# HuttleyLab/DiverseSeq

Hardware: AMD Instinct MI355X
Metric: sequences scored/sec (delta-JSD, k=6) (higher is better)
Workload: dtype f64 (results and every set update in f64; reject/accept decisions tiered: f32 and f32-log scores decide rows farther from the threshold than their proven error bands, f64 the rest)

## Files before the change

diverseseq_amd/csrc/api.cpp:

```cpp
#include "dvs_internal.h"

#include <algorithm>
#include <cmath>
#include <cstring>
#include <mutex>

static std::string g_create_err;

int dvs_set_error(dvs_ctx *ctx, int code, const char *fmt, ...) {
    char buf[512];
    va_list ap;
    va_start(ap, fmt);
    vsnprintf(buf, sizeof buf, fmt, ap);
    va_end(ap);
    if (ctx) ctx->err = buf;
    else g_create_err = buf;
    return code;
}

int dvs_hip_fail(dvs_ctx *ctx, hipError_t e, const char *what) {
    (void)hipGetLastError();
    const int code = (e == hipErrorOutOfMemory) ? DVS_ERR_NOMEM : DVS_ERR_RUNTIME;
    return dvs_set_error(ctx, code, "HIP error %d (%s) in %s", int(e), hipGetErrorString(e), what);
}
// ... 45 lines not shown
int dvs_pinned_get(dvs_ctx *ctx, void **ptr) {
    if (!ctx->pinned_pool.empty()) {
        *ptr = ctx->pinned_pool.back();
        ctx->pinned_pool.pop_back();
        if (__builtin_expect(ctx->knobs.test_poison_blocks, 0)) memset(*ptr, 0xFF, 4096);
        return DVS_OK;
    }
    hipError_t e = hipHostMalloc(ptr, 4096, hipHostMallocDefault);
    if (e != hipSuccess) return dvs_hip_fail(ctx, e, "hipHostMalloc");
    if (__builtin_expect(ctx->knobs.test_poison_blocks, 0)) memset(*ptr, 0xFF, 4096);
    return DVS_OK;
}
void dvs_pinned_put(dvs_ctx *ctx, void *ptr) {
    if (!ptr) return;
    if (ctx) ctx->pinned_pool.push_back(ptr);
    else (void)hipHostFree(ptr);
}
hipEvent_t dvs_event_get(dvs_ctx *ctx) {
    if (!ctx->event_pool.empty()) {
        hipEvent_t e = ctx->event_pool.back();
        ctx->event_pool.pop_back();
        return e;
    }
    hipEvent_t e = nullptr;
    (void)hipEventCreate(&e);
    return e;
}
void dvs_event_put(dvs_ctx *ctx, hipEvent_t e) {
    if (!e) return;
    if (ctx) ctx->event_pool.push_back(e);
// ... 150 lines not shown

void dvs_ctx_release(dvs_ctx *ctx) {
    if (!ctx || --ctx->refs > 0) return;
    (void)hipSetDevice(ctx->device);
    dvs_dev_free(ctx, ctx->off_cache.d_off);
    dvs_dev_free(ctx, ctx->off_cache.d_rows);
    dvs_dev_free(ctx, ctx->off_cache.d_tiles);
    if (ctx->off_cache.ev_up) (void)hipEventDestroy(ctx->off_cache.ev_up);
    if (ctx->off_cache.h_off) (void)hipHostFree(ctx->off_cache.h_off);
    if (ctx->pack_ev) (void)hipEventDestroy(ctx->pack_ev);
    if (ctx->h_pack) (void)hipHostFree(ctx->h_pack);
    dvs_dev_free(ctx, ctx->d_clog_tbl);
    for (auto &kv : ctx->canon_reps) dvs_dev_free(ctx, kv.second);
    dvs_dev_trim(ctx);
    for (void *p : ctx->pinned_pool) (void)hipHostFree(p);
    for (hipEvent_t e : ctx->event_pool) (void)hipEventDestroy(e);
    if (ctx->stream2) (void)hipStreamDestroy(ctx->stream2);
    if (ctx->stream_head) (void)hipStreamDestroy(ctx->stream_head);
    if (ctx->stream_rest) (void)hipStreamDestroy(ctx->stream_rest);
    if (ctx->own_stream && ctx->stream) (void)hipStreamDestroy(ctx->stream);
    delete ctx;
}

extern "C" {

const char *dvs_last_error(const dvs_ctx *ctx) { return ctx ? ctx->err.c_str() : g_create_err.c_str(); }

int dvs_ctx_trim(dvs_ctx *ctx) {
    if (!ctx) return DVS_ERR_VALUE;
    dvs_dev_trim(ctx);
// ... 258 lines not shown
```

diverseseq_amd/csrc/dvs_internal.h:

```cpp
#pragma once

#include <hip/hip_runtime.h>

#include <cstdarg>
#include <cstdint>
#include <cstdio>
#include <functional>
#include <map>
#include <string>
#include <vector>

#include "../../include/dvs_hip.h"

#define DVS_EPS 2.220446049250313e-16
#define DVS_HEAD_ROWS 1024u

struct dvs_knobs {
    bool no_uniform_offsets = false;
    bool no_offsets_cache = false;
    bool counts_u32 = false;
    bool build_wait = false;
    bool no_packed_upload = false;
    bool cu_mask_set = false;
    bool no_fast_step = false;
// ... 25 lines not shown
    int device = 0;
    hipStream_t stream = nullptr;
    bool own_stream = false;
    hipStream_t stream2 = nullptr;
    hipStream_t stream_head = nullptr, stream_rest = nullptr;
    int head_cus = 0;
    bool cu_split_tried = false;
    int persist_timeouts = 0;
    int n_cu = 0;
    size_t lds_per_block = 0;
    double *d_clog_tbl = nullptr;
    bool timing = false;
    std::string err;
    std::multimap<size_t, void *> pool;
    std::vector<void *> pinned_pool;
    std::vector<hipEvent_t> event_pool;
    std::map<void *, size_t> live;
    size_t pool_bytes = 0;
    int refs = 1;
    bool owner_gone = false;
    std::map<const void *, size_t> lds_raised;
    std::map<std::pair<const void *, size_t>, bool> persist_fits;
    struct OffsetsCache {
        uint64_t *h_off = nullptr;
        size_t h_cap = 0, n_off = 0;
        hipEvent_t ev_up = nullptr;
        std::vector<uint32_t> h_long_rows;
        std::vector<unsigned char> h_tiles;
        uint64_t nbytes = 0;
        uint32_t k = 0;
// ... 18 lines not shown
struct dvs_matrix;
int dvs_matrix_settle(dvs_ctx *ctx, const dvs_matrix *m);
int dvs_dev_alloc(dvs_ctx *ctx, void **ptr, size_t bytes, const char *what);
void dvs_dev_free(dvs_ctx *ctx, void *ptr);
void dvs_dev_trim(dvs_ctx *ctx);
struct PooledBuf {
    dvs_ctx *ctx;
    void *p = nullptr;
    ~PooledBuf() { dvs_dev_free(ctx, p); }
    template <typename T>
    T *as() { return static_cast<T *>(p); }
};
int dvs_pinned_get(dvs_ctx *ctx, void **ptr);
int dvs_pinned_stage(dvs_ctx *ctx, size_t bytes, const char *what);
void dvs_pinned_put(dvs_ctx *ctx, void *ptr);
hipEvent_t dvs_event_get(dvs_ctx *ctx);
void dvs_event_put(dvs_ctx *ctx, hipEvent_t e);

int dvs_set_error(dvs_ctx *ctx, int code, const char *fmt, ...);
int dvs_hip_fail(dvs_ctx *ctx, hipError_t e, const char *what);

#define DVS_HIP(ctx, call)                                        \
    do {                                                          \
        hipError_t e__ = (call);                                  \
        if (e__ != hipSuccess) return dvs_hip_fail(ctx, e__, #call); \
    } while (0)

struct dvs_matrix {
    int kind = 0;
    uint16_t *d_counts16 = nullptr;
// ... 312 lines not shown
```

diverseseq_amd/csrc/persist.hip:

```cpp
#include "persist_scan.h"
#include "persist_probe.h"

#include <algorithm>
#include <type_traits>
#include <cstddef>
#include <cstdlib>
#include <cstring>

namespace {

template <typename T, bool CACHED, bool MAXM = false, bool SMALL = false>
__global__ __launch_bounds__(P_THREADS, 2) void persist_nmost_kernel(SelDev d, const T *__restrict__ mat,
                                                                    PSync *sync, unsigned long long *part, uint32_t G) {
    static_assert(!SMALL || (CACHED && !MAXM && sizeof(T) == 2), "SMALL: nmost, 16-bit rows, state in the register cache");
    constexpr uint32_t maxn = SMALL ? P_SMALLN : p_maxn(CACHED, MAXM);
    constexpr bool SPEC = CACHED && !MAXM && sizeof(T) <= 4;
    constexpr bool SPEC_BIG = !CACHED && !MAXM && sizeof(T) <= 4;
    constexpr bool OWN = SPEC && !SMALL;
    extern __shared__ __attribute__((aligned(16))) unsigned char smem[];
    const uint64_t B0 = d.B;
    const uint64_t B = B0;
    double *sl = reinterpret_cast<double *>(smem);
    constexpr bool COARSE = CACHED && sizeof(T) <= 4;
    float *slf = reinterpret_cast<float *>(sl + ((B + 1) & ~1ull));
// ... 50 lines not shown
    st.max_size = MAXM ? ctl->max_size : st.n;
    st.stat = ctl->stat;
    st.mean_d = ctl->mean_delta;
    st.std_d = ctl->std_delta;
    st.cov_d = ctl->cov_delta;
    if (lead && tid == 0) ctl->rows_before_launch = ctl->rows_scored;
    if (ctl->status != SEL_RUN || ctl->ev_kind != 0 || st.n > maxn || st.n < 2) {
        if (lead && tid == 0 && ctl->status == SEL_RUN) ctl->why[7]++;
        return;
    }
    if (MAXM && st.n < st.max_size && (ctl->s_is_resum == 0 || st.n + 2 > maxn)) {
        if (lead && tid == 0) ctl->why[6]++;
        return;
    }
    const bool seeded = !MAXM && CACHED && sync->seeded != 0u;
    for (uint32_t r = tid; r < st.n; r += P_THREADS) {
        const uint32_t slot = seeded ? r : d.ord[r];
        const uint64_t mp = seeded ? sync->seed_list[r] : d.mPos[slot];
        const double t = double(d.totals[mp]);
        s_slot[r] = slot;
        s_mH[r] = seeded ? d.rowH[mp] : d.mH[slot];
        s_pos[r] = mp;
        s_tot[r] = t;
        s_rt[r] = 1.0 / t;
    }
    __syncthreads();
    if (!seeded) {
        const double *low = d.M + uint64_t(s_slot[st.li]) * B;
        const double rn0 = 1.0 / double(st.n);
        for (uint64_t i = tid; i < B; i += P_THREADS) {
// ... 257 lines not shown
        for (uint32_t r = 0; r < st.n; r++) {
            const T *mrow = mat + s_pos[r] * B;
            T cv[P_J];
#pragma unroll
            for (int j = 0; j < P_J; j++) cv[j] = mrow[uint64_t(j) * P_THREADS + tid];
            uint4 q;
            q.x = uint32_t(cv[0]) | (uint32_t(cv[1]) << 16);
            q.y = uint32_t(cv[2]) | (uint32_t(cv[3]) << 16);
            q.z = uint32_t(cv[4]) | (uint32_t(cv[5]) << 16);
            q.w = uint32_t(cv[6]) | (uint32_t(cv[7]) << 16);
            *reinterpret_cast<uint4 *>(s_rows + uint64_t(s_slot[r]) * 4096 + uint32_t(tid) * 8) = q;
        }
    }
    if (sync->no_coarse & 2u) st.thr = 1e300;
#ifdef DVS_PERSIST_STAMPS
    unsigned long long *s_dbg = reinterpret_cast<unsigned long long *>(smem + sync->lds_bytes - 128);
    if (tid < 16) s_dbg[tid] = 0ull;
    __syncthreads();
    unsigned long long t_prev = __builtin_amdgcn_s_memrealtime();
#endif
    for (;;) {
        uint64_t B = B0;
        int tid = tid0;
        asm volatile("" : "+s"(B));
        asm volatile("" : "+v"(tid));
        const uint32_t lane = uint32_t(tid) & 63u, wave = uint32_t(tid) >> 6;
        if (epoch >= P_EPOCH_MAX) {
            bail = true;
            break;
        }
        PRel *myrel = &sync->rel[blockIdx.x & 7u];
// ... 1513 lines not shown
    }

#ifdef DVS_PERSIST_STAMPS
#ifdef DVS_PROBE
    if ((blockIdx.x == n_work - 1 || blockIdx.x == 0) && tid == 0)
        for (int k_ = 0; k_ < 16; k_++) (blockIdx.x == 0 ? sync->dbg2 : sync->dbg)[k_] += s_dbg[k_];
#else
    if ((lead || blockIdx.x == 0) && tid == 0)
        for (int k_ = 0; k_ < 16; k_++) (lead ? sync->dbg : sync->dbg2)[k_] += s_dbg[k_];
#endif
#endif
    if (lead && exit_status != SEL_ERROR && !(exit_status == SEL_ARBITER && arb_stage == ARB_FINALIZE)) {
        const double dn_x = double(st.n);
        for (uint64_t i = tid; i < B; i += P_THREADS) d.base[i] = sl[i] / dn_x;
    }
    if (lane == 0 && nread) {
        atomicAdd(&ctl->rows_scored, (unsigned long long)nread);
        if (nprecise) atomicAdd(&ctl->rows_rechecked, (unsigned long long)nprecise);
        if (nmid) atomicAdd(&ctl->rows_coarse_passed, (unsigned long long)nmid);
    }
    if (lead && tid == 0) {
        ctl->cursor = st.cursor;
        ctl->window = st.window < ctl->window_max ? st.window : ctl->window_max;
        ctl->n_windows += st.n_windows;
        ctl->n_events += st.n_events;
        ctl->n_accepts += st.n_accepts;
        ctl->ev_kind = pend_kind;
        if (exit_status == SEL_ARBITER) {
            ctl->arb_stage = arb_stage;
            ctl->arb_pos = arb_pos;
            if (arb_stage == ARB_RESOLVE) ctl->event_pos = arb_pos;
        }
        ctl->status = (bail || (head_phase && exit_status == SEL_DONE)) ? SEL_RUN
                      : (exit_status == SEL_RUN ? SEL_ERROR : exit_status);
// ... 154 lines not shown
}

}

template <typename T>
static const void *persist_fn(const dvs_select *s) {
    const bool cached = s->dev.B <= uint64_t(P_J) * P_THREADS;
    if (s->params.mode == DVS_MODE_MAX) return reinterpret_cast<const void *>(persist_nmost_kernel<T, true, true>);
    if constexpr (std::is_same_v<T, uint16_t>) {
        if (s->persist.small) return reinterpret_cast<const void *>(persist_nmost_kernel<T, true, false, true>);
    }
    return cached ? reinterpret_cast<const void *>(persist_nmost_kernel<T, true>)
                  : reinterpret_cast<const void *>(persist_nmost_kernel<T, false>);
}

static int persist_prepare(dvs_ctx *ctx, dvs_select *s, uint32_t head_stop, hipStream_t on) {
    std::vector<unsigned char> &image = head_stop ? s->persist.h_sync_head : s->persist.h_sync;
    image.assign(sizeof(PSync), 0);
    PSync &init = *reinterpret_cast<PSync *>(image.data());
    init.stop_at = head_stop;
    init.seeded = s->persist.seeded ? 1u : 0u;
    init.seed_list = static_cast<const unsigned long long *>(s->d_seed_list);
    for (int g = 0; g < 8; g++) init.rel[g].hint = ~0ull;
    init.wg_thresh = s->params.window ? 0u : 4u;
    init.wg_scale = 1.5f;
    if (ctx->knobs.persist_wg_rounds >= 0) init.wg_thresh = uint32_t(ctx->knobs.persist_wg_rounds);
    init.no_coarse = (ctx->knobs.persist_no_coarse ? 1u : 0u) | (ctx->knobs.persist_no_events ? 2u : 0u);
    init.small_rows = s->persist.small ? s->persist.small_rows : 0u;
    init.lds_bytes = uint32_t(s->persist.lds);
    init.wmax = uint32_t(std::min<uint64_t>(s->npos, 0xFFFFFFFFull));
    DVS_HIP(ctx, hipMemcpyAsync(head_stop ? s->persist.sync_head : s->persist.sync, &init, sizeof init, hipMemcpyHostToDevice, on));
    DVS_HIP(ctx, hipMemsetAsync(head_stop ? s->persist.part_head : s->persist.part, 0, p_acc_bytes(s->persist.maxn), on));
    return DVS_OK;
}

template <typename T>
static int persist_launch(dvs_ctx *ctx, dvs_select *s, const T *mat, uint32_t grid, uint32_t head_stop,
                          hipStream_t on) {
    const SelDev &d = s->dev;
    if (head_stop ? !s->persist.head_prepared : !s->persist.prepared) {
        int prc = persist_prepare(ctx, s, head_stop, on);
        if (prc) return prc;
    }
    if (head_stop) s->persist.head_prepared = false;
    else s->persist.prepared = false;
    s->persist.seeded = false;
    const hipEvent_t e1 = dvs_scan_timing_start(ctx, s, on);
// ... 44 lines not shown
        return persist_fn<T>(s);
    });
    int rc = dvs_raise_dyn_lds(ctx, fn, lds);
    if (rc) return rc;
    {
        auto key = std::make_pair(fn, lds);
        auto hit = ctx->persist_fits.find(key);
        if (hit == ctx->persist_fits.end()) {
            int per_cu = 0;
            const bool fits = hipOccupancyMaxActiveBlocksPerMultiprocessor(&per_cu, fn, P_THREADS, lds) == hipSuccess && per_cu >= 1;
            if (!fits) (void)hipGetLastError();
            hit = ctx->persist_fits.emplace(key, fits).first;
        }
        if (!hit->second) return DVS_OK;
    }
    rc = dvs_dev_alloc(ctx, &s->persist.sync, sizeof(PSync), "persistent sync block");
    if (!rc) rc = dvs_dev_alloc(ctx, &s->persist.part, p_acc_bytes(s->persist.maxn) + (maxm ? 2 * p_batch_bytes() : 0),
                                "leave-one-out accumulators");
    if (rc) return rc;
    s->persist.on = true;
    return DVS_OK;
}

void dvs_persist_free(dvs_select *s) {
    dvs_dev_free(s->ctx, s->persist.sync);
    dvs_dev_free(s->ctx, s->persist.part);
    dvs_dev_free(s->ctx, s->persist.sync_head);
    dvs_dev_free(s->ctx, s->persist.part_head);
}

int dvs_persist_launch(dvs_ctx *ctx, dvs_select *s) {
    return dvs_mat_dispatch(s->mat, [&](auto *mp) { return persist_launch(ctx, s, mp, s->persist.grid, 0u, ctx->stream); });
}

static int persist_head_blocks(dvs_ctx *ctx, dvs_select *s) {
    if (s->persist.sync_head) return DVS_OK;
    int rc = dvs_dev_alloc(ctx, &s->persist.sync_head, sizeof(PSync), "head phase sync block");
    if (!rc) rc = dvs_dev_alloc(ctx, &s->persist.part_head, p_acc_bytes(s->persist.maxn), "head phase accumulators");
    return rc;
}

int dvs_persist_launch_head(dvs_ctx *ctx, dvs_select *s, uint32_t grid, uint32_t stop_at, hipStream_t on) {
    int rc = persist_head_blocks(ctx, s);
    if (rc) return rc;
    return dvs_mat_dispatch(s->mat, [&](auto *mp) { return persist_launch(ctx, s, mp, grid, stop_at, on); });
}

int dvs_persist_prepare_head(dvs_ctx *ctx, dvs_select *s, uint32_t stop_at, hipStream_t on) {
    int rc = persist_head_blocks(ctx, s);
    if (!rc) rc = persist_prepare(ctx, s, stop_at, on);
    if (!rc) s->persist.head_prepared = true;
    return rc;
}
// ... 43 lines not shown
```

diverseseq_amd/csrc/persist_dev.h:

```cpp
#pragma once

#include "select_dev.h"

namespace {

constexpr int P_THREADS = 512;
constexpr int P_J = 8;
constexpr int P_CH = 16;
constexpr uint32_t P_MAXN = 512;
constexpr uint32_t P_MAXN_BIG = 256;
constexpr uint32_t P_MAXN_MAX = 896;
constexpr uint32_t p_maxn(bool cached, bool maxm = false) { return cached ? (maxm ? P_MAXN_MAX : P_MAXN) : P_MAXN_BIG; }
constexpr uint32_t P_SMALLN = 16;
constexpr uint32_t P_SMALL_ROWS = 13;
constexpr uint32_t p_maxjobs(bool cached, bool maxm = false) { return p_maxn(cached, maxm) + 1; }
constexpr size_t p_acc_bytes(uint32_t maxn) { return size_t(8) * (maxn + 1) * 2 * sizeof(unsigned long long); }
__device__ __forceinline__ unsigned long long p_acc_word(double v) {
    return ((unsigned long long)__double2ll_rn(v * 0x1p50) << 6) + 1ull;
}
__device__ __forceinline__ double p_acc_value(unsigned long long w) { return double((long long)w >> 6) * 0x1p-50; }
__device__ __forceinline__ void p_acc_add(unsigned long long *dst, double th, double ts) {
    atomicAdd(dst, p_acc_word(th));
    atomicAdd(dst + 1, p_acc_word(ts));
}
// ... 12 lines not shown
        v = __hip_atomic_load(w, __ATOMIC_RELAXED, __HIP_MEMORY_SCOPE_AGENT);
    }
    *prev = v;
    return v - before;
}
constexpr uint32_t P_SPIN_LIMIT = 1u << 22;
constexpr uint32_t P_MAXG = 256;
constexpr uint32_t P_FLAT_GRID = 64;
constexpr uint32_t P_WINWORDS = 64;
constexpr uint32_t P_LIST = 2;
constexpr uint32_t P_BATCH = 32;
constexpr uint32_t P_BATCH_MEMBERS = 256;
constexpr size_t p_batch_bytes() { return size_t(P_BATCH) * (P_BATCH_MEMBERS + 2) * 4 * sizeof(double); }
constexpr size_t p_batch_lds() { return size_t(P_BATCH) * (2 + 12 + 24) * sizeof(double); }

constexpr size_t P_LDS_SLACK = 56;
constexpr size_t P_LDS_SLACK_SMALL = 16;
constexpr size_t p_lds_bytes(uint64_t B, int kind, bool cached, bool maxm, uint32_t small_rows) {
    const bool coarse = cached && kind != 1, own = coarse && !maxm && !small_rows;
    const size_t maxn = small_rows ? P_SMALLN : p_maxn(cached, maxm);
    const size_t sl = ((B + 1) & ~1ull) * sizeof(double);
    const size_t slf = coarse ? ((B + 3) & ~3ull) * sizeof(float) : 0;
    const size_t Sl = maxm ? sl : 0;
    const size_t scratch = 128 * sizeof(double);
    const size_t members = maxn * (5 * sizeof(double) + sizeof(uint64_t) + sizeof(uint32_t));
    const size_t s_win = P_WINWORDS * sizeof(unsigned long long), flags = 16, s_ltab = 128 * sizeof(double2);
    const size_t s_prev = (maxn + 1) * 2 * sizeof(unsigned long long);
    const size_t tail = maxm         ? p_batch_lds()
                        : small_rows ? small_rows * B * sizeof(uint16_t) + P_LDS_SLACK_SMALL
                        : own        ? maxn * sizeof(uint32_t) + size_t(P_J) * P_THREADS * (kind == 2 ? sizeof(uint16_t) : sizeof(uint32_t))
                                     : 0;
    const size_t stamps = 128;
    return sl + slf + Sl + scratch + members + s_win + flags + s_ltab + s_prev + tail + stamps + P_LDS_SLACK;
}
static_assert(p_lds_bytes(4096, 2, true, false, 2) == 70440 && p_lds_bytes(4096, 2, true, false, 13) == 160552, "nmost, 4096 bins, 16-bit, SMALL");
static_assert(p_lds_bytes(4096, 2, true, false, 0) == 98008, "nmost, 4096 bins, 16-bit, OWN");
static_assert(p_lds_bytes(4096, 0, true, false, 0) == 106200 && p_lds_bytes(4096, 1, true, false, 0) == 71384, "nmost, 4096 bins, 32-bit and f64");
static_assert(p_lds_bytes(16384, 2, false, false, 0) == 152280 && p_lds_bytes(16384, 0, false, false, 0) == 152280, "nmost, 16384 bins");
static_assert(p_lds_bytes(4096, 2, true, true, 0) == 156376 && p_lds_bytes(256, 2, true, true, 0) == 79576, "max, 16-bit");
static_assert(p_lds_bytes(125, 0, true, false, 0) == 58568, "nmost, 125 bins, 32-bit");

struct PLine {
    uint32_t v;
    uint32_t pad[63];
};
struct PRel {
    unsigned long long rel;
    unsigned long long hint;
// ... 14 lines not shown
    const unsigned long long *seed_list;
    uint32_t small_rows;
    uint32_t lds_bytes;
    uint32_t wmax;
    uint32_t pad2[53];
    PRel rel[8];
    unsigned long long wrec[2][P_MAXG];
    unsigned long long soft[2][P_MAXG][P_LIST];
#ifdef DVS_PERSIST_STAMPS
    unsigned long long trace[4][8][P_MAXG];
#endif
    unsigned long long dbg2[16];
    unsigned long long dbg[16];
};

struct PState {
    uint64_t cursor, npos;
    uint32_t window, wmin, wmax;
    uint32_t n, li;
    double sumH, total_jsd, thr, band, wscale;
    uint32_t n_windows, n_events, n_accepts;
    uint32_t max_size, stat;
    double mean_d, std_d, cov_d;
};

#define RLX_AGENT __ATOMIC_RELAXED, __HIP_MEMORY_SCOPE_AGENT

constexpr uint32_t P_TAG0 = 0xFFFFFEu;
constexpr uint32_t P_EPOCH_MAX = 0xFFFFF0u;
constexpr unsigned long long P_POS_NONE = (1ull << 37) - 1;
// ... 216 lines not shown
```

diverseseq_amd/csrc/select.h:

```cpp
#pragma once

#include "dvs_internal.h"

#define SEL_NONE 0xFFFFFFFFFFFFFFFFull
#define SEL_SEEDS_AT 512

enum : uint32_t { SEL_RUN = 0, SEL_DONE = 1, SEL_ARBITER = 2, SEL_ERROR = 3,
                  SEL_NEED_SETUP = 4 };
enum : uint32_t { ARB_RESOLVE = 1, ARB_FINALIZE = 2 };
enum : uint32_t { FORCE_NONE = 0, FORCE_ACCEPT = 1, FORCE_REJECT = 2, FORCE_COMMIT = 3, FORCE_ROLLBACK = 4 };

struct SelCtl {
    unsigned long long cursor;
    unsigned long long npos;
    unsigned long long event_pos;
    unsigned long long arb_pos;
    unsigned long long rows_scored, rows_rechecked;
    unsigned long long rows_coarse_passed;
    unsigned long long rows_before_launch;
    uint32_t window, window_min, window_max;
    uint32_t status, arb_stage, forced, forced_lowest;
    uint32_t size, lowest, mode, max_size, stat;
    uint32_t ev_kind;
    uint32_t ev_n;
// ... 32 lines not shown
    double *dtmp = nullptr;
    double *dsum = nullptr;
    uint32_t *mLabel = nullptr;
    unsigned long long *mPos = nullptr;
    uint32_t *ord = nullptr;
    uint8_t *inset = nullptr;
    uint32_t *wg_rows = nullptr;
    unsigned long long *evlog_pos = nullptr;
    uint32_t *evlog_kind = nullptr;
    const double *gather_all = nullptr;
    uint32_t gather_world = 0;
    double *rowlog = nullptr;
    uint32_t rowlog_cap = 0;
};

struct dvs_select {
    dvs_ctx *ctx = nullptr;
    dvs_select_params params{};
    const dvs_matrix *mat = nullptr;
    int mat_kind = 0;
    uint64_t npos = 0;
    uint32_t cap = 0;
    SelDev dev;
    SelCtl *h_ctl = nullptr;
    SelCtl ctl0{};
    std::vector<uint32_t> h_order, h_labels;
    std::vector<uint32_t> h_out_labels;
    std::vector<uint64_t> seed_positions;
    uint32_t scan_grid = 0, loo_grid = 0;
    size_t scan_lds = 0;
    bool base_in_lds = true;
    bool scan_hot = false;
    struct {
        bool on = false;
        uint32_t grid = 0, maxn = 0, maxjobs = 0;
        bool small = false;
        uint32_t small_rows = 0;
        size_t lds = 0;
        void *sync = nullptr;
        std::vector<unsigned char> h_sync;
        std::vector<unsigned char> h_sync_head;
        void *part = nullptr;
        void *sync_head = nullptr, *part_head = nullptr;
        bool seeded = false;
        bool head_prepared = false;
        bool prepared = false;
    } persist;
    struct {
        double *d_res = nullptr;
        uint32_t jw = 0;
        uint32_t launched = 0;
    } mb;
    bool seeded_start = false;
    bool used_side_streams = false;
    hipEvent_t ev_side_done = nullptr;
    void *d_seed_list = nullptr;
    bool seed_list_in_ctl = false;
    bool inset_clean = false;
    hipStream_t setup_side = nullptr;
    bool head_phase = false;
    int batch = 16;
    bool time_scan = false;
    std::vector<hipEvent_t> ev_pool;
    size_t ev_used = 0;
    double scan_ms = 0.0;
    double scan_ms_last = 0.0;
    uint64_t scan_launches = 0;
    uint32_t n_arbitrated = 0;
    double arbiter_ms = 0.0;
// ... 13 lines not shown
        uint64_t rowlog_have = 0;
        uint32_t steps_since_poll = 0;
    } fs;
    void *arbiter = nullptr;
};

int dvs_select_arbitrate(dvs_ctx *ctx, dvs_select *s);
void dvs_select_arbiter_free(dvs_select *s);

int dvs_persist_setup(dvs_ctx *ctx, dvs_select *s);
void dvs_persist_free(dvs_select *s);
int dvs_persist_launch(dvs_ctx *ctx, dvs_select *s);
int dvs_persist_launch_head(dvs_ctx *ctx, dvs_select *s, uint32_t grid, uint32_t stop_at, hipStream_t on);
int dvs_persist_prepare_main(dvs_ctx *ctx, dvs_select *s);
int dvs_persist_prepare_head(dvs_ctx *ctx, dvs_select *s, uint32_t stop_at, hipStream_t on);
void dvs_persist_debug_report(dvs_ctx *ctx, const dvs_select *s);
void dvs_persist_debug_done(const SelCtl &c);

hipEvent_t dvs_scan_timing_start(dvs_ctx *ctx, dvs_select *s, hipStream_t on);
void dvs_select_launch_scan(dvs_ctx *ctx, dvs_select *s, bool hot);
void dvs_select_launch_iteration(dvs_ctx *ctx, dvs_select *s, int stage);
int dvs_select_poll(dvs_ctx *ctx, dvs_select *s);
int dvs_select_arbitrate_resume(dvs_ctx *ctx, dvs_select *s);

int dvs_stepwise_alloc(dvs_ctx *ctx, dvs_select *s, const uint32_t *labels);
void dvs_stepwise_wait(dvs_select *s);
void dvs_stepwise_free(dvs_select *s);
#ifdef DVS_FS_TRACE
void dvs_stepwise_trace_report(const dvs_select *s);
#endif
// ... 4 lines not shown
```

diverseseq_amd/csrc/select.hip:

```cpp
#include "dvs_internal.h"
#include "select.h"
#include "select_dev.h"

#include <algorithm>
#include <chrono>
#include <type_traits>
#include <cmath>
#include <cstring>
#include <cstdlib>
#include <memory>

namespace {

constexpr int SCAN_THREADS = 512;

template <typename T>
__device__ __forceinline__ void scan_rows_hot(SelCtl *ctl, const T *__restrict__ mat,
                                              const uint32_t *__restrict__ totals,
                                              const double *__restrict__ rowH, const double *bvec,
                                              uint64_t B, const ScanState &st, uint64_t first,
                                              uint64_t stride, uint32_t lane, uint32_t &nread,
                                              uint32_t &nprecise) {
    for (uint64_t r = first; r < st.nrows; r += stride) {
        const uint64_t p = st.cursor + r;
// ... 685 lines not shown
        for (uint64_t i = threadIdx.x; i < d.B; i += LOO_THREADS) out[i] = 0.0;
        if (threadIdx.x == 0) meta[2 * r] = meta[2 * r + 1] = 0.0;
        return;
    }
    const uint32_t slot = d.ord[r];
    const double *src = d.M + uint64_t(slot) * d.B;
    for (uint64_t i = threadIdx.x; i < d.B; i += LOO_THREADS) out[i] = src[i];
    if (threadIdx.x == 0) {
        meta[2 * r] = double(d.mPos[slot]);
        meta[2 * r + 1] = 1.0;
    }
}

}

static void sel_free(dvs_select *s) {
    if (!s) return;
#ifdef DVS_FS_TRACE
    dvs_stepwise_trace_report(s);
#endif
    if (s->used_side_streams && s->ctx) {
        if (s->ctx->stream_head) (void)hipStreamSynchronize(s->ctx->stream_head);
        if (s->ctx->stream2) (void)hipStreamSynchronize(s->ctx->stream2);
    }
    void *ptrs[] = {s->dev.ctl, s->dev.S, s->dev.Stmp, s->dev.base, s->dev.cand, s->dev.M,
                    s->dev.mH, s->dev.mDelta, s->dev.dtmp, s->dev.dsum, s->dev.mLabel, s->dev.mPos,
                    s->dev.ord, s->dev.inset, s->dev.wg_rows, s->dev.evlog_pos, s->dev.evlog_kind, s->dev.rowlog,
                    (void *)s->dev.order, (void *)s->dev.labels};
    for (void *p : ptrs)
        dvs_dev_free(s->ctx, p);
    dvs_stepwise_wait(s);
    dvs_pinned_put(s->ctx, s->h_ctl);
    for (hipEvent_t e : s->ev_pool) dvs_event_put(s->ctx, e);
    dvs_max_batch_free(s);
    dvs_stepwise_free(s);
    dvs_persist_free(s);
    if (!s->seed_list_in_ctl) dvs_dev_free(s->ctx, s->d_seed_list);
    if (s->ev_side_done) dvs_event_put(s->ctx, s->ev_side_done);
    dvs_select_arbiter_free(s);
    dvs_ctx_release(s->ctx);
    delete s;
}
// ... 48 lines not shown
    hipLaunchKernelGGL(finalize_kernel, dim3(1), dim3(WIDE_THREADS), 0, stream, d);
}

void dvs_select_launch_scan(dvs_ctx *ctx, dvs_select *s, bool hot) {
    dvs_mat_dispatch(s->mat, [&](auto *mp) { launch_scan(s, mp, hot, s->dev.ctl, s->dev.wg_rows, ctx->stream); return 0; });
}
void dvs_select_launch_iteration(dvs_ctx *ctx, dvs_select *s, int stage) {
    dvs_mat_dispatch(s->mat, [&](auto *mp) { launch_iteration(ctx, s, mp, stage); return 0; });
}

int dvs_select_poll(dvs_ctx *ctx, dvs_select *s) {
    DVS_HIP(ctx, hipMemcpyAsync(s->h_ctl, s->dev.ctl, sizeof(SelCtl), hipMemcpyDeviceToHost,
                                ctx->stream));
    DVS_HIP(ctx, hipStreamSynchronize(ctx->stream));
    const_cast<dvs_matrix *>(s->mat)->in_flight = false;
    return DVS_OK;
}

template <typename T>
static int sel_seed(dvs_ctx *ctx, dvs_select *s, const T *mat, hipStream_t st, bool light = false);

template <typename T>
static int sel_drop_seeded(dvs_ctx *ctx, dvs_select *s, const T *mat, hipStream_t st) {
    s->seeded_start = false;
    s->persist.seeded = false;
    return sel_seed<T>(ctx, s, mat, st);
}

template <typename T>
static int sel_leave_persist(dvs_ctx *ctx, dvs_select *s, const T *mat, bool restart) {
// ... 123 lines not shown
    if (s->mat->head_rows_built && s->params.n_seed <= s->mat->head_rows_built && s->h_order.empty() &&
        !(s->params.flags & DVS_SELECT_STEPWISE)) {
        s->head_phase = s->mat->rest_beside_head && ctx->stream_head && s->persist.on &&
                        s->params.mode == DVS_MODE_NMOST && s->params.window == 0 &&
                        s->cap + 2 <= uint32_t(ctx->head_cus) && s->npos > 4ull * s->mat->head_rows_built &&
                        s->params.n_seed + 64 <= s->mat->head_rows_built && !ctx->knobs.no_head_phase;
        s->setup_side = s->head_phase ? ctx->stream_head : dvs_ctx_stream2(ctx);
    }
}

template <typename T>
static int sel_start(dvs_ctx *ctx, dvs_select *s, const T *mat) {
    hipStream_t side = s->setup_side;
    const bool head_phase = s->head_phase;
    hipStream_t st = side ? side : ctx->stream;
    if (side) s->used_side_streams = true;
    int rc = sel_seed<T>(ctx, s, mat, st, s->seeded_start);
    if (rc) return rc;
    if (head_phase) {
        rc = dvs_persist_launch_head(ctx, s, uint32_t(ctx->head_cus), s->mat->head_rows_built, side);
        if (rc == DVS_ERR_UNSUPPORTED)
            rc = s->seeded_start ? sel_drop_seeded<T>(ctx, s, mat, st) : DVS_OK;
        if (rc) return rc;
        rc = dvs_persist_prepare_main(ctx, s);
        if (rc) return rc;
        const_cast<dvs_matrix *>(s->mat)->rest_beside_head = false;
    }
    if (side) {
        if (!s->ev_side_done) s->ev_side_done = dvs_event_get(ctx);
        DVS_HIP(ctx, hipEventRecord(s->ev_side_done, side));
        DVS_HIP(ctx, hipStreamWaitEvent(ctx->stream, s->ev_side_done, 0));
    }
    if (s->params.flags & DVS_SELECT_STEPWISE) return dvs_select_poll(ctx, s);
    return sel_run_loop<T>(ctx, s, mat);
}

template <typename T>
static int sel_seed(dvs_ctx *ctx, dvs_select *s, const T *mat, hipStream_t st, bool light) {
    const std::vector<uint64_t> &seeds = s->seed_positions;
    SelDev &d = s->dev;
    SelCtl c = s->ctl0;
    const uint32_t wdef = s->params.window ? s->params.window : (s->persist.on ? s->persist.grid * 2u : 4096u);
    c.window_min = wdef;
    c.window_max = std::max<uint32_t>(wdef, s->scan_grid * (SCAN_THREADS / 64) * 8);
    c.window = wdef;
    *s->h_ctl = c;
// ... 127 lines not shown
    const struct { void **ptr; size_t bytes; const char *what; } blocks[] = {
        {(void **)&d.ctl, 4096, "d.ctl"},
        {(void **)&d.S, B * 8, "d.S"},
        {(void **)&d.Stmp, B * 8, "d.Stmp"},
        {(void **)&d.base, B * 8, "d.base"},
        {(void **)&d.cand, B * 8, "d.cand"},
        {(void **)&d.M, size_t(cap) * B * 8, "d.M"},
        {(void **)&d.mH, size_t(cap) * 8, "d.mH"},
        {(void **)&d.mDelta, size_t(cap) * 8, "d.mDelta"},
        {(void **)&d.dtmp, size_t(cap) * 8, "d.dtmp"},
        {(void **)&d.dsum, size_t(cap) * 8, "d.dsum"},
        {(void **)&d.mLabel, size_t(cap) * 4, "d.mLabel"},
        {(void **)&d.mPos, size_t(cap) * 8, "d.mPos"},
        {(void **)&d.ord, size_t(cap) * 4, "d.ord"},
        {(void **)&d.inset, std::max<size_t>(nlabels, 1), "d.inset"},
        {(void **)&d.wg_rows, size_t(s->scan_grid) * 8, "d.wg_rows"},
        {(void **)&d.evlog_pos, nlog * 8, "d.evlog_pos"},
        {(void **)&d.evlog_kind, nlog * 4, "d.evlog_kind"},
    };
    for (const auto &b : blocks)
        if (int rc = dvs_dev_alloc(ctx, b.ptr, b.bytes, b.what)) return rc;
    if (s->params.flags & DVS_SELECT_STEPWISE)
        if (int rc = dvs_stepwise_alloc(ctx, s, labels)) return rc;
    if (order) {
        if (int rc = dvs_dev_alloc(ctx, (void **)&d.order, size_t(npos) * 4, "d.order")) return rc;
        DVS_HIP(ctx, hipMemcpyAsync((void *)d.order, order, size_t(npos) * 4, hipMemcpyHostToDevice, ctx->stream));
    }
    if (labels) {
        if (int rc = dvs_dev_alloc(ctx, (void **)&d.labels, size_t(npos) * 4, "d.labels")) return rc;
        DVS_HIP(ctx, hipMemcpyAsync((void *)d.labels, labels, size_t(npos) * 4, hipMemcpyHostToDevice, ctx->stream));
    }
    static_assert(sizeof(SelCtl) <= 4096, "control block must fit a cached pinned block");
    return dvs_pinned_get(ctx, (void **)&s->h_ctl);
}

static int sel_prepare_engine(dvs_ctx *ctx, dvs_select *s, const uint32_t *order, const uint32_t *labels) {
    SelDev &d = s->dev;
    const dvs_matrix *m = s->mat;
    const uint32_t n_seed = s->params.n_seed, nlabels = d.nlabels;
    int rc = dvs_persist_setup(ctx, s);
    if (rc) return rc;
    sel_plan_setup_stream(ctx, s);
    if (s->setup_side) s->used_side_streams = true;
    DVS_HIP(ctx, hipMemsetAsync(d.inset, 0, std::max<size_t>(nlabels, 1), s->setup_side ? s->setup_side : ctx->stream));
    s->inset_clean = true;
    DVS_HIP(ctx, hipMemsetAsync(d.wg_rows, 0, size_t(s->scan_grid) * 8, s->setup_side ? s->setup_side : ctx->stream));
    s->seeded_start = s->persist.on && s->params.mode == DVS_MODE_NMOST && d.B <= 4096 && !order && !labels &&
                      !(s->params.flags & DVS_SELECT_STEPWISE) && n_seed >= 2 && n_seed <= 32 && !ctx->knobs.persist_no_seeded;
    s->persist.seeded = s->seeded_start;
    if (size_t(n_seed) * sizeof(uint64_t) <= 4096 - SEL_SEEDS_AT) {
        s->d_seed_list = reinterpret_cast<unsigned char *>(d.ctl) + SEL_SEEDS_AT;
        s->seed_list_in_ctl = true;
    } else if (s->seeded_start) {
        if ((rc = dvs_dev_alloc(ctx, &s->d_seed_list, size_t(n_seed) * sizeof(uint64_t), "seed list"))) return rc;
    }
    if (s->persist.on && m->rest_beside_head && ctx->stream_head && m->head_rows_built && s->params.mode == DVS_MODE_NMOST &&
        !order && !labels) {
        s->used_side_streams = true;
        return dvs_persist_prepare_head(ctx, s, m->head_rows_built, ctx->stream_head);
    }
    return DVS_OK;
}

static int sel_read_seeds(dvs_ctx *ctx, dvs_select *s, const uint32_t *order) {
    const dvs_matrix *m = s->mat;
    const uint32_t n_seed = s->params.n_seed;
    std::vector<uint32_t> h_tot(n_seed);
    int rc = dvs_matrix_settle(ctx, m);
    if (rc) return rc;
    hipError_t ce = hipSuccess;
    if (!order && n_seed && n_seed <= m->h_head_totals.size()) {
        std::copy(m->h_head_totals.begin(), m->h_head_totals.begin() + n_seed, h_tot.begin());
    } else if (!order && n_seed) {
// ... 239 lines not shown
```

Before: 69.94 million.

## Merge persistent launch blocks into one pinned upload and aggregate exit counters per workgroup

The sync block, the accumulators and (for the head phase) the wg_rows scratch now sit in one device allocation. Each is initialised by a single async copy from a cached, pre-zeroed pinned host image, replacing a separate memcpy plus memsets. Kernel exit counters are first summed in LDS per workgroup, so only one global atomic per counter is issued per workgroup. Side-stream synchronisation at free is skipped for streams already joined, and the head phase reuses its timing event as the join point. The cost is more state tracking, such as pending-upload flags and side-stream bitmasks, plus a change to the LDS layout.

```diff
diff --git a/diverseseq_amd/csrc/api.cpp b/diverseseq_amd/csrc/api.cpp
--- a/diverseseq_amd/csrc/api.cpp
+++ b/diverseseq_amd/csrc/api.cpp
@@ -83,6 +83,27 @@
 void dvs_pinned_put(dvs_ctx *ctx, void *ptr) {
     if (!ptr) return;
     if (ctx) ctx->pinned_pool.push_back(ptr);
+    else (void)hipHostFree(ptr);
+}
+int dvs_pinned_image_get(dvs_ctx *ctx, size_t bytes, void **ptr) {
+    const size_t sz = ((bytes ? bytes : 1) + 4095) & ~size_t(4095);
+    auto it = ctx->pinned_images.find(sz);
+    if (it != ctx->pinned_images.end()) {
+        *ptr = it->second;
+        ctx->pinned_images.erase(it);
+    } else {
+        const hipError_t e = hipHostMalloc(ptr, sz, hipHostMallocDefault);
+        if (e != hipSuccess) {
+            *ptr = nullptr;
+            return dvs_hip_fail(ctx, e, "pinned image of a launch block");
+        }
+    }
+    if (__builtin_expect(ctx->knobs.test_poison_blocks, 0)) memset(*ptr, 0xFF, sz);
+    return DVS_OK;
+}
+void dvs_pinned_image_put(dvs_ctx *ctx, void *ptr, size_t bytes) {
+    if (!ptr) return;
+    if (ctx) ctx->pinned_images.emplace(((bytes ? bytes : 1) + 4095) & ~size_t(4095), ptr);
     else (void)hipHostFree(ptr);
 }
 hipEvent_t dvs_event_get(dvs_ctx *ctx) {
@@ -263,6 +284,7 @@
     for (auto &kv : ctx->canon_reps) dvs_dev_free(ctx, kv.second);
     dvs_dev_trim(ctx);
     for (void *p : ctx->pinned_pool) (void)hipHostFree(p);
+    for (auto &kv : ctx->pinned_images) (void)hipHostFree(kv.second);
     for (hipEvent_t e : ctx->event_pool) (void)hipEventDestroy(e);
     if (ctx->stream2) (void)hipStreamDestroy(ctx->stream2);
     if (ctx->stream_head) (void)hipStreamDestroy(ctx->stream_head);
diff --git a/diverseseq_amd/csrc/dvs_internal.h b/diverseseq_amd/csrc/dvs_internal.h
--- a/diverseseq_amd/csrc/dvs_internal.h
+++ b/diverseseq_amd/csrc/dvs_internal.h
@@ -63,6 +63,7 @@
     std::string err;
     std::multimap<size_t, void *> pool;
     std::vector<void *> pinned_pool;
+    std::multimap<size_t, void *> pinned_images;
     std::vector<hipEvent_t> event_pool;
     std::map<void *, size_t> live;
     size_t pool_bytes = 0;
@@ -111,6 +112,8 @@
 int dvs_pinned_get(dvs_ctx *ctx, void **ptr);
 int dvs_pinned_stage(dvs_ctx *ctx, size_t bytes, const char *what);
 void dvs_pinned_put(dvs_ctx *ctx, void *ptr);
+int dvs_pinned_image_get(dvs_ctx *ctx, size_t bytes, void **ptr);
+void dvs_pinned_image_put(dvs_ctx *ctx, void *ptr, size_t bytes);
 hipEvent_t dvs_event_get(dvs_ctx *ctx);
 void dvs_event_put(dvs_ctx *ctx, hipEvent_t e);
 
diff --git a/diverseseq_amd/csrc/persist.hip b/diverseseq_amd/csrc/persist.hip
--- a/diverseseq_amd/csrc/persist.hip
+++ b/diverseseq_amd/csrc/persist.hip
@@ -88,6 +88,7 @@
         return;
     }
     const bool seeded = !MAXM && CACHED && sync->seeded != 0u;
+    if (tid < 4) p_exit_words(smem, sync)[tid] = 0ull;
     for (uint32_t r = tid; r < st.n; r += P_THREADS) {
         const uint32_t slot = seeded ? r : d.ord[r];
         const uint64_t mp = seeded ? sync->seed_list[r] : d.mPos[slot];
@@ -375,7 +376,7 @@
     }
     if (sync->no_coarse & 2u) st.thr = 1e300;
 #ifdef DVS_PERSIST_STAMPS
-    unsigned long long *s_dbg = reinterpret_cast<unsigned long long *>(smem + sync->lds_bytes - 128);
+    unsigned long long *s_dbg = reinterpret_cast<unsigned long long *>(smem + sync->lds_bytes - P_LDS_STAMPS);
     if (tid < 16) s_dbg[tid] = 0ull;
     __syncthreads();
     unsigned long long t_prev = __builtin_amdgcn_s_memrealtime();
@@ -1919,10 +1920,20 @@
         const double dn_x = double(st.n);
         for (uint64_t i = tid; i < B; i += P_THREADS) d.base[i] = sl[i] / dn_x;
     }
-    if (lane == 0 && nread) {
-        atomicAdd(&ctl->rows_scored, (unsigned long long)nread);
-        if (nprecise) atomicAdd(&ctl->rows_rechecked, (unsigned long long)nprecise);
-        if (nmid) atomicAdd(&ctl->rows_coarse_passed, (unsigned long long)nmid);
+    if (lane == 0) {
+        unsigned long long *s_exit = p_exit_words(smem, sync);
+        if (nread) atomicAdd(&s_exit[0], (unsigned long long)nread);
+        if (nprecise) atomicAdd(&s_exit[1], (unsigned long long)nprecise);
+        if (nmid) atomicAdd(&s_exit[2], (unsigned long long)nmid);
+        const unsigned long long before = __hip_atomic_fetch_add(&s_exit[3], 1ull, __ATOMIC_ACQ_REL, __HIP_MEMORY_SCOPE_WORKGROUP);
+        if (before == P_THREADS / 64 - 1) {
+            const unsigned long long wg_read = __hip_atomic_load(&s_exit[0], __ATOMIC_RELAXED, __HIP_MEMORY_SCOPE_WORKGROUP);
+            const unsigned long long wg_precise = __hip_atomic_load(&s_exit[1], __ATOMIC_RELAXED, __HIP_MEMORY_SCOPE_WORKGROUP);
+            const unsigned long long wg_mid = __hip_atomic_load(&s_exit[2], __ATOMIC_RELAXED, __HIP_MEMORY_SCOPE_WORKGROUP);
+            if (wg_read) atomicAdd(&ctl->rows_scored, wg_read);
+            if (wg_precise) atomicAdd(&ctl->rows_rechecked, wg_precise);
+            if (wg_mid) atomicAdd(&ctl->rows_coarse_passed, wg_mid);
+        }
     }
     if (lead && tid == 0) {
         ctl->cursor = st.cursor;
@@ -2107,23 +2118,35 @@
                   : reinterpret_cast<const void *>(persist_nmost_kernel<T, false>);
 }
 
+static size_t p_block_acc_at() { return (sizeof(PSync) + 255) & ~size_t(255); }
+static size_t p_block_tail_at(uint32_t maxn) { return p_block_acc_at() + p_acc_bytes(maxn); }
+
 static int persist_prepare(dvs_ctx *ctx, dvs_select *s, uint32_t head_stop, hipStream_t on) {
-    std::vector<unsigned char> &image = head_stop ? s->persist.h_sync_head : s->persist.h_sync;
-    image.assign(sizeof(PSync), 0);
-    PSync &init = *reinterpret_cast<PSync *>(image.data());
+    auto &ps = s->persist;
+    void *&image = head_stop ? ps.h_image_head : ps.h_image;
+    size_t &bytes = head_stop ? ps.image_head_bytes : ps.image_bytes;
+    bool &zeroed = head_stop ? ps.image_head_zeroed : ps.image_zeroed;
+    if (!image) {
+        bytes = p_block_tail_at(ps.maxn) + (head_stop ? ps.head_tail : 0);
+        if (int rc = dvs_pinned_image_get(ctx, bytes, &image)) return rc;
+        zeroed = false;
+    }
+    std::memset(image, 0, zeroed ? sizeof(PSync) : bytes);
+    zeroed = true;
+    PSync &init = *static_cast<PSync *>(image);
     init.stop_at = head_stop;
-    init.seeded = s->persist.seeded ? 1u : 0u;
+    init.seeded = ps.seeded ? 1u : 0u;
     init.seed_list = static_cast<const unsigned long long *>(s->d_seed_list);
     for (int g = 0; g < 8; g++) init.rel[g].hint = ~0ull;
     init.wg_thresh = s->params.window ? 0u : 4u;
     init.wg_scale = 1.5f;
     if (ctx->knobs.persist_wg_rounds >= 0) init.wg_thresh = uint32_t(ctx->knobs.persist_wg_rounds);
     init.no_coarse = (ctx->knobs.persist_no_coarse ? 1u : 0u) | (ctx->knobs.persist_no_events ? 2u : 0u);
-    init.small_rows = s->persist.small ? s->persist.small_rows : 0u;
-    init.lds_bytes = uint32_t(s->persist.lds);
+    init.small_rows = ps.small ? ps.small_rows : 0u;
+    init.lds_bytes = uint32_t(ps.lds);
     init.wmax = uint32_t(std::min<uint64_t>(s->npos, 0xFFFFFFFFull));
-    DVS_HIP(ctx, hipMemcpyAsync(head_stop ? s->persist.sync_head : s->persist.sync, &init, sizeof init, hipMemcpyHostToDevice, on));
-    DVS_HIP(ctx, hipMemsetAsync(head_stop ? s->persist.part_head : s->persist.part, 0, p_acc_bytes(s->persist.maxn), on));
+    if (on == ctx->stream) ps.upload_pending = true;
+    DVS_HIP(ctx, hipMemcpyAsync(head_stop ? ps.sync_head : ps.sync, image, bytes, hipMemcpyHostToDevice, on));
     return DVS_OK;
 }
 
@@ -2198,19 +2221,22 @@
         }
         if (!hit->second) return DVS_OK;
     }
-    rc = dvs_dev_alloc(ctx, &s->persist.sync, sizeof(PSync), "persistent sync block");
-    if (!rc) rc = dvs_dev_alloc(ctx, &s->persist.part, p_acc_bytes(s->persist.maxn) + (maxm ? 2 * p_batch_bytes() : 0),
-                                "leave-one-out accumulators");
+    rc = dvs_dev_alloc(ctx, &s->persist.sync, p_block_tail_at(s->persist.maxn) + (maxm ? 2 * p_batch_bytes() : 0),
+                       "persistent launch block");
     if (rc) return rc;
+    s->persist.part = static_cast<unsigned char *>(s->persist.sync) + p_block_acc_at();
     s->persist.on = true;
     return DVS_OK;
 }
 
 void dvs_persist_free(dvs_select *s) {
+    if (s->persist.upload_pending && s->ctx) (void)hipStreamSynchronize(s->ctx->stream);
+    s->persist.upload_pending = false;
     dvs_dev_free(s->ctx, s->persist.sync);
-    dvs_dev_free(s->ctx, s->persist.part);
     dvs_dev_free(s->ctx, s->persist.sync_head);
-    dvs_dev_free(s->ctx, s->persist.part_head);
+    dvs_pinned_image_put(s->ctx, s->persist.h_image, s->persist.image_bytes);
+    dvs_pinned_image_put(s->ctx, s->persist.h_image_head, s->persist.image_head_bytes);
+    s->persist.h_image = s->persist.h_image_head = nullptr;
 }
 
 int dvs_persist_launch(dvs_ctx *ctx, dvs_select *s) {
@@ -2219,8 +2245,17 @@
 
 static int persist_head_blocks(dvs_ctx *ctx, dvs_select *s) {
     if (s->persist.sync_head) return DVS_OK;
-    int rc = dvs_dev_alloc(ctx, &s->persist.sync_head, sizeof(PSync), "head phase sync block");
-    if (!rc) rc = dvs_dev_alloc(ctx, &s->persist.part_head, p_acc_bytes(s->persist.maxn), "head phase accumulators");
+    const int rc = dvs_dev_alloc(ctx, &s->persist.sync_head, p_block_tail_at(s->persist.maxn) + s->persist.head_tail,
+                                 "head phase launch block");
+    if (!rc) s->persist.part_head = static_cast<unsigned char *>(s->persist.sync_head) + p_block_acc_at();
+    return rc;
+}
+
+int dvs_persist_head_tail(dvs_ctx *ctx, dvs_select *s, size_t bytes, void **tail) {
+    if (s->persist.sync_head) return dvs_set_error(ctx, DVS_ERR_RUNTIME, "the head phase's block exists already");
+    s->persist.head_tail = bytes;
+    const int rc = persist_head_blocks(ctx, s);
+    if (!rc) *tail = static_cast<unsigned char *>(s->persist.sync_head) + p_block_tail_at(s->persist.maxn);
     return rc;
 }
 
diff --git a/diverseseq_amd/csrc/persist_dev.h b/diverseseq_amd/csrc/persist_dev.h
--- a/diverseseq_amd/csrc/persist_dev.h
+++ b/diverseseq_amd/csrc/persist_dev.h
@@ -50,7 +50,9 @@
 constexpr size_t p_batch_bytes() { return size_t(P_BATCH) * (P_BATCH_MEMBERS + 2) * 4 * sizeof(double); }
 constexpr size_t p_batch_lds() { return size_t(P_BATCH) * (2 + 12 + 24) * sizeof(double); }
 
-constexpr size_t P_LDS_SLACK = 56;
+constexpr size_t P_LDS_EXIT = 32;
+constexpr size_t P_LDS_STAMPS = 128;
+constexpr size_t P_LDS_SLACK = 24;
 constexpr size_t P_LDS_SLACK_SMALL = 16;
 constexpr size_t p_lds_bytes(uint64_t B, int kind, bool cached, bool maxm, uint32_t small_rows) {
     const bool coarse = cached && kind != 1, own = coarse && !maxm && !small_rows;
@@ -66,8 +68,7 @@
                         : small_rows ? small_rows * B * sizeof(uint16_t) + P_LDS_SLACK_SMALL
                         : own        ? maxn * sizeof(uint32_t) + size_t(P_J) * P_THREADS * (kind == 2 ? sizeof(uint16_t) : sizeof(uint32_t))
                                      : 0;
-    const size_t stamps = 128;
-    return sl + slf + Sl + scratch + members + s_win + flags + s_ltab + s_prev + tail + stamps + P_LDS_SLACK;
+    return sl + slf + Sl + scratch + members + s_win + flags + s_ltab + s_prev + tail + P_LDS_SLACK + P_LDS_EXIT + P_LDS_STAMPS;
 }
 static_assert(p_lds_bytes(4096, 2, true, false, 2) == 70440 && p_lds_bytes(4096, 2, true, false, 13) == 160552, "nmost, 4096 bins, 16-bit, SMALL");
 static_assert(p_lds_bytes(4096, 2, true, false, 0) == 98008, "nmost, 4096 bins, 16-bit, OWN");
@@ -112,6 +113,10 @@
     unsigned long long dbg[16];
 };
 
+__device__ __forceinline__ unsigned long long *p_exit_words(unsigned char *smem, const PSync *sync) {
+    return reinterpret_cast<unsigned long long *>(smem + sync->lds_bytes - (P_LDS_STAMPS + P_LDS_EXIT));
+}
+
 struct PState {
     uint64_t cursor, npos;
     uint32_t window, wmin, wmax;
diff --git a/diverseseq_amd/csrc/select.h b/diverseseq_amd/csrc/select.h
--- a/diverseseq_amd/csrc/select.h
+++ b/diverseseq_amd/csrc/select.h
@@ -70,6 +70,8 @@
     uint32_t rowlog_cap = 0;
 };
 
+constexpr uint8_t SEL_SIDE_HEAD = 1, SEL_SIDE_2 = 2;
+
 struct dvs_select {
     dvs_ctx *ctx = nullptr;
     dvs_select_params params{};
@@ -94,10 +96,14 @@
         uint32_t small_rows = 0;
         size_t lds = 0;
         void *sync = nullptr;
-        std::vector<unsigned char> h_sync;
-        std::vector<unsigned char> h_sync_head;
         void *part = nullptr;
         void *sync_head = nullptr, *part_head = nullptr;
+        void *h_image = nullptr, *h_image_head = nullptr;
+        size_t image_bytes = 0, image_head_bytes = 0;
+        bool image_zeroed = false, image_head_zeroed = false;
+        bool upload_pending = false;
+        size_t head_tail = 0;
+        bool wg_rows_in_head = false;
         bool seeded = false;
         bool head_prepared = false;
         bool prepared = false;
@@ -109,6 +115,7 @@
     } mb;
     bool seeded_start = false;
     bool used_side_streams = false;
+    uint8_t side_open = 0, side_joined = 0;
     hipEvent_t ev_side_done = nullptr;
     void *d_seed_list = nullptr;
     bool seed_list_in_ctl = false;
@@ -152,6 +159,7 @@
 int dvs_persist_launch_head(dvs_ctx *ctx, dvs_select *s, uint32_t grid, uint32_t stop_at, hipStream_t on);
 int dvs_persist_prepare_main(dvs_ctx *ctx, dvs_select *s);
 int dvs_persist_prepare_head(dvs_ctx *ctx, dvs_select *s, uint32_t stop_at, hipStream_t on);
+int dvs_persist_head_tail(dvs_ctx *ctx, dvs_select *s, size_t bytes, void **tail);
 void dvs_persist_debug_report(dvs_ctx *ctx, const dvs_select *s);
 void dvs_persist_debug_done(const SelCtl &c);
 
diff --git a/diverseseq_amd/csrc/select.hip b/diverseseq_amd/csrc/select.hip
--- a/diverseseq_amd/csrc/select.hip
+++ b/diverseseq_amd/csrc/select.hip
@@ -723,18 +723,25 @@
 
 }
 
+static void sel_side_queued(dvs_ctx *ctx, dvs_select *s, hipStream_t st) {
+    const uint8_t bit = st == ctx->stream_head ? SEL_SIDE_HEAD : SEL_SIDE_2;
+    s->used_side_streams = true;
+    s->side_open |= bit;
+    s->side_joined &= uint8_t(~bit);
+}
+
 static void sel_free(dvs_select *s) {
     if (!s) return;
 #ifdef DVS_FS_TRACE
     dvs_stepwise_trace_report(s);
 #endif
     if (s->used_side_streams && s->ctx) {
-        if (s->ctx->stream_head) (void)hipStreamSynchronize(s->ctx->stream_head);
-        if (s->ctx->stream2) (void)hipStreamSynchronize(s->ctx->stream2);
+        if (s->ctx->stream_head && (s->side_open & SEL_SIDE_HEAD)) (void)hipStreamSynchronize(s->ctx->stream_head);
+        if (s->ctx->stream2 && (s->side_open & SEL_SIDE_2)) (void)hipStreamSynchronize(s->ctx->stream2);
     }
     void *ptrs[] = {s->dev.ctl, s->dev.S, s->dev.Stmp, s->dev.base, s->dev.cand, s->dev.M,
                     s->dev.mH, s->dev.mDelta, s->dev.dtmp, s->dev.dsum, s->dev.mLabel, s->dev.mPos,
-                    s->dev.ord, s->dev.inset, s->dev.wg_rows, s->dev.evlog_pos, s->dev.evlog_kind, s->dev.rowlog,
+                    s->dev.ord, s->dev.inset, s->persist.wg_rows_in_head ? nullptr : s->dev.wg_rows, s->dev.evlog_pos, s->dev.evlog_kind, s->dev.rowlog,
                     (void *)s->dev.order, (void *)s->dev.labels};
     for (void *p : ptrs)
         dvs_dev_free(s->ctx, p);
@@ -813,6 +820,11 @@
                                 ctx->stream));
     DVS_HIP(ctx, hipStreamSynchronize(ctx->stream));
     const_cast<dvs_matrix *>(s->mat)->in_flight = false;
+    s->persist.upload_pending = false;
+    if (s->side_joined && (s->h_ctl->status == SEL_DONE || s->h_ctl->status == SEL_RUN)) {
+        s->side_open &= uint8_t(~s->side_joined);
+        s->side_joined = 0;
+    }
     return DVS_OK;
 }
 
@@ -966,11 +978,13 @@
     hipStream_t side = s->setup_side;
     const bool head_phase = s->head_phase;
     hipStream_t st = side ? side : ctx->stream;
-    if (side) s->used_side_streams = true;
+    if (side) sel_side_queued(ctx, s, side);
     int rc = sel_seed<T>(ctx, s, mat, st, s->seeded_start);
     if (rc) return rc;
+    hipEvent_t side_end = nullptr;
     if (head_phase) {
         rc = dvs_persist_launch_head(ctx, s, uint32_t(ctx->head_cus), s->mat->head_rows_built, side);
+        if (rc == DVS_OK && s->time_scan && s->ev_used >= 2) side_end = s->ev_pool[s->ev_used - 1];
         if (rc == DVS_ERR_UNSUPPORTED)
             rc = s->seeded_start ? sel_drop_seeded<T>(ctx, s, mat, st) : DVS_OK;
         if (rc) return rc;
@@ -979,9 +993,13 @@
         const_cast<dvs_matrix *>(s->mat)->rest_beside_head = false;
     }
     if (side) {
-        if (!s->ev_side_done) s->ev_side_done = dvs_event_get(ctx);
-        DVS_HIP(ctx, hipEventRecord(s->ev_side_done, side));
-        DVS_HIP(ctx, hipStreamWaitEvent(ctx->stream, s->ev_side_done, 0));
+        if (!side_end) {
+            if (!s->ev_side_done) s->ev_side_done = dvs_event_get(ctx);
+            DVS_HIP(ctx, hipEventRecord(s->ev_side_done, side));
+            side_end = s->ev_side_done;
+        }
+        DVS_HIP(ctx, hipStreamWaitEvent(ctx->stream, side_end, 0));
+        s->side_joined |= side == ctx->stream_head ? SEL_SIDE_HEAD : SEL_SIDE_2;
     }
     if (s->params.flags & DVS_SELECT_STEPWISE) return dvs_select_poll(ctx, s);
     return sel_run_loop<T>(ctx, s, mat);
@@ -1139,7 +1157,6 @@
         {(void **)&d.mPos, size_t(cap) * 8, "d.mPos"},
         {(void **)&d.ord, size_t(cap) * 4, "d.ord"},
         {(void **)&d.inset, std::max<size_t>(nlabels, 1), "d.inset"},
-        {(void **)&d.wg_rows, size_t(s->scan_grid) * 8, "d.wg_rows"},
         {(void **)&d.evlog_pos, nlog * 8, "d.evlog_pos"},
         {(void **)&d.evlog_kind, nlog * 4, "d.evlog_kind"},
     };
@@ -1166,10 +1183,20 @@
     int rc = dvs_persist_setup(ctx, s);
     if (rc) return rc;
     sel_plan_setup_stream(ctx, s);
-    if (s->setup_side) s->used_side_streams = true;
+    if (s->setup_side) sel_side_queued(ctx, s, s->setup_side);
     DVS_HIP(ctx, hipMemsetAsync(d.inset, 0, std::max<size_t>(nlabels, 1), s->setup_side ? s->setup_side : ctx->stream));
     s->inset_clean = true;
-    DVS_HIP(ctx, hipMemsetAsync(d.wg_rows, 0, size_t(s->scan_grid) * 8, s->setup_side ? s->setup_side : ctx->stream));
+    const bool head_block = s->persist.on && m->rest_beside_head && ctx->stream_head && m->head_rows_built &&
+                            s->params.mode == DVS_MODE_NMOST && !order && !labels;
+    if (head_block && s->setup_side == ctx->stream_head) {
+        void *tail = nullptr;
+        if ((rc = dvs_persist_head_tail(ctx, s, size_t(s->scan_grid) * 8, &tail))) return rc;
+        d.wg_rows = static_cast<uint32_t *>(tail);
+        s->persist.wg_rows_in_head = true;
+    } else {
+        if ((rc = dvs_dev_alloc(ctx, (void **)&d.wg_rows, size_t(s->scan_grid) * 8, "d.wg_rows"))) return rc;
+        DVS_HIP(ctx, hipMemsetAsync(d.wg_rows, 0, size_t(s->scan_grid) * 8, s->setup_side ? s->setup_side : ctx->stream));
+    }
     s->seeded_start = s->persist.on && s->params.mode == DVS_MODE_NMOST && d.B <= 4096 && !order && !labels &&
                       !(s->params.flags & DVS_SELECT_STEPWISE) && n_seed >= 2 && n_seed <= 32 && !ctx->knobs.persist_no_seeded;
     s->persist.seeded = s->seeded_start;
@@ -1179,9 +1206,8 @@
     } else if (s->seeded_start) {
         if ((rc = dvs_dev_alloc(ctx, &s->d_seed_list, size_t(n_seed) * sizeof(uint64_t), "seed list"))) return rc;
     }
-    if (s->persist.on && m->rest_beside_head && ctx->stream_head && m->head_rows_built && s->params.mode == DVS_MODE_NMOST &&
-        !order && !labels) {
-        s->used_side_streams = true;
+    if (head_block) {
+        sel_side_queued(ctx, s, ctx->stream_head);
         return dvs_persist_prepare_head(ctx, s, m->head_rows_built, ctx->stream_head);
     }
     return DVS_OK;
```

Result: faster. 72.01 million, median of 6 (+3.0%).
